# FireMines/zk_stark_project

Hardware: AMD Instinct MI355X
Metric: STARK proofs/sec + prove-time ms, MiMC AIR 2^20-step trace (higher is better)
Workload: dtype f128 (u128 mod 2^128-45*2^40+1); 1 GPU; MiMC AIR 2^20-step trace, blowup=8 (BASELINE configs[1]); trace_length=1048576, trace_width=1, blowup=8, num_queries=40, grinding=21, fri_folding=16, fri_remainder_max_degree=7, parallelism=replicas1

## Files before the change

zk_stark_project_amd/csrc/merkle.hip:

```cpp
#include "kernels_dev.hpp"
#include "blake3_quad.hpp"

#include <cstdlib>

using kc::rev_bits;
using kc::static_for;

namespace {

struct MerkleArgs {
  const felt* src;
  uint64_t n;
  uint32_t cols;
  uint32_t logB;
  uint64_t R;
  uint32_t* nodes;
  uint64_t L;
  MerkleTail tail;
  LastCol lc;
  GuLazy gl;
};

__device__ __forceinline__ felt gu_lazy_value(const GuLazy& gl, const felt* base, const felt* prev, uint64_t cstride,
                                              felt l, uint32_t c) {
// ... 183 lines not shown
      uint32_t l[8], r[8];
#pragma unroll
      for (int i = 0; i < 8; i++) { l[i] = sd[(2 * t) * 9 + i]; r[i] = sd[(2 * t + 1) * 9 + i]; }
      merge8(l, r, o);
    }
    __syncthreads();
    if (t < s) {
#pragma unroll
      for (int i = 0; i < 8; i++) sd[t * 9 + i] = o[i];
      store_digest(nodes + (first + t) * 8, o);
    }
  }
}

__device__ __forceinline__ void merkle_tail_op(const MerkleTail& tl, const uint32_t* root);

template <int MODE, bool QUAD = false>
__global__ __launch_bounds__(256) void k_merkle_fused(MerkleArgs a) {
  __shared__ uint32_t sd[256 * 9];
  const uint32_t t = threadIdx.x;
  const uint64_t L = a.L;
  constexpr uint64_t LB = QUAD ? 64 : 512;
  const uint64_t cnt = L < LB ? L : LB;
  const uint64_t base = (uint64_t)blockIdx.x * LB;
  uint64_t first;
  uint32_t s0;
  if constexpr (QUAD) {
    const uint32_t nd = t >> 2, q = t & 3;
    if (nd < cnt) {
      uint32_t o0, o1;
// ... 9 lines not shown
      merkle_leaf<MODE>(a, base + 2 * t, d0);
      merkle_leaf<MODE>(a, base + 2 * t + 1, d1);
      if (MODE != 2) {
        store_digest(a.nodes + (L + base + 2 * t) * 8, d0);
        store_digest(a.nodes + (L + base + 2 * t + 1) * 8, d1);
      }
      merge8(d0, d1, m);
      store_digest(a.nodes + ((L >> 1) + (base >> 1) + t) * 8, m);
#pragma unroll
      for (int i = 0; i < 8; i++) sd[t * 9 + i] = m[i];
    }
    first = (L >> 1) + (base >> 1);
    s0 = (uint32_t)(cnt >> 2);
  }
  lds_levels(sd, s0, a.nodes, first);
  if (!a.tail.done) return;
  __shared__ int s_last;
  __threadfence();
  __syncthreads();
  if (t == 0) s_last = atomicAdd(a.tail.done, 1u) == gridDim.x - 1;
  __syncthreads();
  if (!s_last) return;
  __threadfence();
  const uint32_t G = gridDim.x;
  if (G > 1) {
    if (G / 2 <= 64) {
      const uint32_t nd = t >> 2, q = t & 3;
      if (t < 4 * (G / 2)) {
        uint32_t mm[16], o0, o1;
        const uint32_t* src = a.nodes + (uint64_t)(G + 2 * nd) * 8;
#pragma unroll
        for (int k = 0; k < 16; k++) mm[k] = src[k];
        merge_quad(mm, q, o0, o1);
        quad_store(sd, a.nodes + (uint64_t)(G / 2 + nd) * 8, nd, q, o0, o1);
      }
    } else {
      for (uint32_t i = t; i < G / 2; i += 256) {
        uint32_t l[8], r[8], o[8];
        load_digest(a.nodes + (uint64_t)(G + 2 * i) * 8, l);
        load_digest(a.nodes + (uint64_t)(G + 2 * i + 1) * 8, r);
        merge8(l, r, o);
        store_digest(a.nodes + (uint64_t)(G / 2 + i) * 8, o);
#pragma unroll
        for (int k = 0; k < 8; k++) sd[i * 9 + k] = o[k];
      }
    }
    lds_levels(sd, G / 4, a.nodes, G / 2);
  }
  __syncthreads();
  if (t == 0) *a.tail.done = 0;
  if (a.tail.op != MERKLE_TAIL_NONE) merkle_tail_op(a.tail, a.nodes + 8);
}
// ... 382 lines not shown
  seed[4 + q] = s1;
  root_out[q] = r[q];
  root_out[4 + q] = r[4 + q];
}

__global__ void k_coin_fri_layer(uint32_t* __restrict__ seed, const uint32_t* __restrict__ root,
                                 felt* __restrict__ alpha_out, uint32_t* __restrict__ root_out) {
  if (blockIdx.x != 0) return;
  coin_fri_step(seed, root, alpha_out, root_out);
}

struct SeedArg {
  uint32_t w[8];
};

__global__ __launch_bounds__(TPB) void k_pack(PackArgs a, uint32_t* __restrict__ dst) {
  const uint32_t seg = blockIdx.y;
  if (seg >= a.n) return;
  const uint32_t* src = reinterpret_cast<const uint32_t*>(a.src[seg]);
  const uint64_t words = a.bytes[seg] / 4, o = a.off[seg] / 4;
  for (uint64_t i = blockIdx.x * (uint64_t)TPB + threadIdx.x; i < words; i += (uint64_t)gridDim.x * TPB)
    dst[o + i] = src[i];
}

__device__ __forceinline__ felt shfl_down_felt(felt v, int d) {
  const int a = __shfl_down((int)(uint32_t)v.lo, d), b = __shfl_down((int)(uint32_t)(v.lo >> 32), d);
  const int c = __shfl_down((int)(uint32_t)v.hi, d), e = __shfl_down((int)(uint32_t)(v.hi >> 32), d);
  return fp::make((uint64_t)(uint32_t)a | ((uint64_t)(uint32_t)b << 32),
                  (uint64_t)(uint32_t)c | ((uint64_t)(uint32_t)e << 32));
}
__device__ __forceinline__ void remainder_coeffs_block(const felt* __restrict__ E, uint32_t logB, uint32_t m,
                                                       uint32_t ncoef, felt off_inv, felt wd_inv, felt d_inv,
                                                       felt* s_c, felt* s_tw) {
  const uint32_t D = m << logB, t = threadIdx.x, lane = t & 63, wave = t >> 6, nw = blockDim.x >> 6;
  for (uint32_t j = t; j < D; j += blockDim.x) s_tw[j] = fp::pow_u64(wd_inv, j);
  __syncthreads();
  for (uint32_t k = wave; k < ncoef; k += nw) {
// ... 34 lines not shown
  uint32_t m[16];
#pragma unroll
  for (int k = 0; k < 8; k++) m[k] = seedp ? seedp[k] : seed.w[k];
  m[8] = (uint32_t)nonce;
  m[9] = (uint32_t)(nonce >> 32);
#pragma unroll
  for (int k = 10; k < 16; k++) m[k] = 0;
  uint32_t out[8];
  b3::set_iv(out);
  b3::compress(out, m, 0, 40, b3::CHUNK_START | b3::CHUNK_END | b3::ROOT);
  uint64_t h = (uint64_t)out[0] | ((uint64_t)out[1] << 32);
  uint32_t tz = h == 0 ? 64u : (uint32_t)__builtin_ctzll(h);
  if (tz >= bits) atomicMin(result, (unsigned long long)nonce);
}

__global__ __launch_bounds__(TPB) void k_grind_all(const uint32_t* __restrict__ seedp, uint64_t base, uint64_t limit,
                                                   uint32_t bits, unsigned long long* result) {
  const uint64_t T = (uint64_t)gridDim.x * TPB, g = blockIdx.x * (uint64_t)TPB + threadIdx.x;
  using b3::rotr;
  uint32_t m[16];
#pragma unroll
  for (int k = 0; k < 8; k++) m[k] = seedp[k];
#pragma unroll
  for (int k = 8; k < 16; k++) m[k] = 0;
  uint32_t p0 = b3::iv(0), p1 = b3::iv(1), p2 = b3::iv(2), p3 = b3::iv(3), p4 = b3::iv(4), p5 = b3::iv(5),
           p6 = b3::iv(6), p7 = b3::iv(7), p8 = b3::iv(0), p9 = b3::iv(1), p10 = b3::iv(2), p11 = b3::iv(3),
           p12 = 0, p13 = 0, p14 = 40, p15 = b3::CHUNK_START | b3::CHUNK_END | b3::ROOT;
  {
#define sp(i) p##i
#define B3_GP(a, b, c, d, x, y)            \
  sp(a) = sp(a) + sp(b) + (x);              \
  sp(d) = rotr(sp(d) ^ sp(a), 16);          \
  sp(c) = sp(c) + sp(d);                    \
  sp(b) = rotr(sp(b) ^ sp(c), 12);          \
  sp(a) = sp(a) + sp(b) + (y);              \
  sp(d) = rotr(sp(d) ^ sp(a), 8);           \
  sp(c) = sp(c) + sp(d);                    \
  sp(b) = rotr(sp(b) ^ sp(c), 7);
    B3_GP(0, 4, 8, 12, m[0], m[1]) B3_GP(1, 5, 9, 13, m[2], m[3])
    B3_GP(2, 6, 10, 14, m[4], m[5]) B3_GP(3, 7, 11, 15, m[6], m[7])
    B3_GP(1, 6, 11, 12, 0u, 0u) B3_GP(2, 7, 8, 13, 0u, 0u) B3_GP(3, 4, 9, 14, 0u, 0u)
#undef B3_GP
#undef sp
  }
  for (uint64_t start = base;; start += T) {
    if (start > limit || __hip_atomic_load(result, __ATOMIC_RELAXED, __HIP_MEMORY_SCOPE_AGENT) < start) return;
    const uint64_t nonce = start + g;
    m[8] = (uint32_t)nonce;
    m[9] = (uint32_t)(nonce >> 32);
    uint32_t s0 = p0, s1 = p1, s2 = p2, s3 = p3, s4 = p4, s5 = p5, s6 = p6, s7 = p7, s8 = p8, s9 = p9, s10 = p10,
             s11 = p11, s12 = p12, s13 = p13, s14 = p14, s15 = p15;
    B3_G(0, 5, 10, 15, m[8], m[9])
    B3_ROUND(2, 6, 3, 10, 7, 0, 4, 13, 1, 11, 12, 5, 9, 14, 15, 8)
    B3_ROUND(3, 4, 10, 12, 13, 2, 7, 14, 6, 5, 9, 0, 11, 15, 8, 1)
    B3_ROUND(10, 7, 12, 9, 14, 3, 13, 15, 4, 0, 11, 2, 5, 8, 1, 6)
    B3_ROUND(12, 13, 9, 11, 15, 10, 14, 8, 7, 2, 5, 3, 0, 1, 6, 4)
    B3_ROUND(9, 14, 11, 5, 8, 12, 15, 1, 13, 3, 0, 10, 2, 6, 4, 7)
    B3_ROUND(11, 15, 5, 0, 1, 9, 8, 6, 14, 10, 2, 12, 3, 4, 7, 13)
    const uint64_t h = (uint64_t)(s0 ^ s8) | ((uint64_t)(s1 ^ s9) << 32);
    const uint32_t tz = h == 0 ? 64u : (uint32_t)__builtin_ctzll(h);
    if (tz >= bits) atomicMin(result, (unsigned long long)nonce);
  }
}

__global__ void k_query_positions(const uint32_t* __restrict__ seedp, const unsigned long long* __restrict__ nonce_p,
                                  uint32_t q, uint64_t N, uint64_t* __restrict__ pos) {
  const uint64_t nonce = *nonce_p;
  uint32_t m[16], s2[8];
#pragma unroll
  for (int k = 0; k < 8; k++) m[k] = seedp[k];
  m[8] = (uint32_t)nonce;
  m[9] = (uint32_t)(nonce >> 32);
#pragma unroll
  for (int k = 10; k < 16; k++) m[k] = 0;
  b3::set_iv(s2);
  b3::compress_r(s2, m, 0, 40, b3::CHUNK_START | b3::CHUNK_END | b3::ROOT);
  for (uint32_t i = threadIdx.x; i < q; i += blockDim.x) {
#pragma unroll
    for (int k = 0; k < 8; k++) m[k] = s2[k];
    m[8] = i + 1;
    m[9] = 0;
#pragma unroll
    for (int k = 10; k < 16; k++) m[k] = 0;
    uint32_t out[8];
    b3::set_iv(out);
    b3::compress_r(out, m, 0, 40, b3::CHUNK_START | b3::CHUNK_END | b3::ROOT);
    pos[i] = ((uint64_t)out[0] | ((uint64_t)out[1] << 32)) & (N - 1);
  }
}

__global__ __launch_bounds__(128) void k_gather_full(FullGatherArgs a, const uint64_t* __restrict__ pos,
                                                     uint32_t* __restrict__ out) {
  const uint32_t i = blockIdx.x, y = blockIdx.y, t = threadIdx.x;
  const uint64_t p = pos[i];
  const uint64_t B = 1ull << a.logB;
  uint32_t* rec = out + a.seg_off[y] + (uint64_t)i * a.rec_words[y];
  if (y == 0) {
    const uint64_t j = p & (B - 1), tt = p >> a.logB;
    const uint32_t nv = a.w + a.C, depth = a.logN;
    for (uint32_t e = t; e < 4 * nv; e += blockDim.x) {
      const uint32_t c = e >> 2;
      const felt* src = c < a.w ? a.tlde + ((uint64_t)c * B + j) * a.n : a.clde + ((uint64_t)(c - a.w) * B + j) * a.n;
      rec[e] = reinterpret_cast<const uint32_t*>(src + tt)[e & 3];
    }
    uint32_t* paths = rec + 4 * nv;
    for (uint32_t e = t; e < 2 * depth * 8; e += blockDim.x) {
      const uint32_t tree = e / (depth * 8), d = (e / 8) % depth, wd = e & 7;
      const uint64_t node = (((1ull << a.logN) + p) >> d) ^ 1ull;
// ... 118 lines not shown
  const uint64_t q = tq >> 2;
  const uint32_t qd = (uint32_t)(tq & 3);
  const felt v = fri_fold_row_quad(E, q < rows ? q : rows - 1, qd, logm16, j0, logB, alpha_p, off_inv, itw_lev,
                                   eps_inv);
  if (q < rows && qd == 0) out[q] = v;
}

template <int F>
__global__ __launch_bounds__(TPB) void k_fri_fold(const felt* __restrict__ E, uint64_t rows, uint32_t logmF,
                                                  uint32_t j0, uint32_t logB, const felt* __restrict__ alpha_p,
                                                  felt off_inv, const felt* __restrict__ itw_lev,
                                                  const felt* __restrict__ eps_inv, felt* __restrict__ out) {
  const uint64_t q = blockIdx.x * (uint64_t)TPB + threadIdx.x;
  if (q >= rows) return;
  out[q] = fri_fold_row_f<F>(E, q, logmF, j0, logB, alpha_p, off_inv, itw_lev, eps_inv);
}

template <int F>
__global__ __launch_bounds__(512) void k_fri_tail(FriTailArgs a) {
  __shared__ uint32_t sd[128 * 9];
  __shared__ felt s_c[256];
  __shared__ felt s_tw[256];
  __shared__ uint32_t s_cv[32][8];
  const uint32_t t = threadIdx.x, nd = t >> 2, q = t & 3;
  for (uint32_t l = 0; l < a.nl; l++) {
    const FriTailLayer y = a.ly[l];
    const uint32_t R = 1u << (y.logm16 + a.logB);
    MerkleArgs ma{};
    ma.src = y.E;
    ma.R = 1ull << y.logm16;
// ... 142 lines not shown
void preload_merkle_module() {
  hipFuncAttributes fa;
  (void)hipFuncGetAttributes(&fa, (const void*)k_coin_fri_layer);
}

void launch_grind(Prof& prof, hipStream_t s, const uint32_t* seed_words, const uint32_t* seed_dev, uint64_t base,
                  uint64_t count, uint32_t bits, unsigned long long* result) {
  SeedArg sa;
  for (int i = 0; i < 8; i++) sa.w[i] = seed_words ? seed_words[i] : 0u;
  LAUNCH(prof, "grind", s, 0.0,
         hipLaunchKernelGGL(k_grind, dim3(blocks_for(count)), dim3(TPB), 0, s, sa, seed_dev, base, count, bits,
                            result));
}

void launch_grind_all(Prof& prof, hipStream_t s, const uint32_t* seed_dev, uint64_t base, uint64_t limit,
                      uint32_t bits, unsigned long long* result) {
  LAUNCH(prof, "grind", s, 0.0,
         hipLaunchKernelGGL(k_grind_all, dim3(1024), dim3(TPB), 0, s, seed_dev, base, limit, bits, result));
}

void launch_query_positions(Prof& prof, hipStream_t s, const uint32_t* seed_dev, const unsigned long long* nonce,
                            uint32_t q, uint64_t N, uint64_t* pos) {
  LAUNCH(prof, "positions", s, 0.0, hipLaunchKernelGGL(k_query_positions, dim3(1), dim3(256), 0, s, seed_dev, nonce, q,
                                                       N, pos));
}

void launch_gather_full(Prof& prof, hipStream_t s, const FullGatherArgs& a, uint32_t q, const uint64_t* pos,
                        uint32_t* out) {
  LAUNCH(prof, "gather", s, 0.0,
         hipLaunchKernelGGL(k_gather_full, dim3(q, 1 + a.nlayers), dim3(128), 0, s, a, pos, out));
}

void launch_pack(Prof& prof, hipStream_t s, const PackArgs& a, void* dst) {
  uint64_t mx = 0;
  for (uint32_t i = 0; i < a.n; i++) mx = a.bytes[i] > mx ? a.bytes[i] : mx;
  const uint32_t bx = (uint32_t)std::min<uint64_t>(std::max<uint64_t>((mx / 4 + TPB - 1) / TPB, 1), 64);
  LAUNCH(prof, "gather", s, 0.0,
         hipLaunchKernelGGL(k_pack, dim3(bx, a.n), dim3(TPB), 0, s, a, reinterpret_cast<uint32_t*>(dst)));
}

void launch_fri_remainder(Prof& prof, hipStream_t s, const felt* E, uint32_t logB, uint32_t m, felt off_inv,
                          felt wd_inv, felt d_inv, uint32_t* seed, felt* rem_out, uint32_t* commit_out) {
  const uint32_t D = m << logB, ncoef = m;
  if (D > 256) launch_fail(ZKP_ERR_DEVICE, "internal: device remainder over 256 values");
  LAUNCH(prof, "coin", s, 0.0,
// ... 15 lines not shown
  const uint64_t rows = m16 * Bl;
  if (F == 16 && rows <= (1ull << 15)) {
    LAUNCH(prof, "fri_fold16", s, (double)rows * (16 * 16.0 + 16.0),
           hipLaunchKernelGGL(k_fri_fold16_quad, dim3(blocks_for(rows * 4)), dim3(TPB), 0, s, E, rows, logm16, j0,
                              logB, alpha, off_inv, lev, eps_inv, out));
    return;
  }
#define ZKP_FOLD(FF)                                                                                             \
  case FF:                                                                                                       \
    LAUNCH(prof, "fri_fold" #FF, s, (double)rows * (FF * 16.0 + 16.0),                                           \
           hipLaunchKernelGGL(k_fri_fold<FF>, dim3(blocks_for(rows)), dim3(TPB), 0, s, E, rows, logm16, j0, logB, \
                              alpha, off_inv, lev, eps_inv, out));                                               \
    return;
  switch (F) { ZKP_FOLD(2) ZKP_FOLD(4) ZKP_FOLD(8) ZKP_FOLD(16) }
#undef ZKP_FOLD
  launch_fail(ZKP_ERR_DEVICE, "internal: FRI folding factor");
}

void launch_fri_tail(Prof& prof, hipStream_t s, const FriTailArgs& a) {
  if (a.nl > FRI_TAIL_MAX || (a.rem_m << a.logB) > 256) launch_fail(ZKP_ERR_DEVICE, "internal: FRI tail shape");
  for (uint32_t l = 0; l < a.nl; l++) {
    const uint32_t logrows = a.ly[l].logm16 + a.logB;
    if (logrows > 7)
      launch_fail(ZKP_ERR_DEVICE, "internal: FRI tail layer over 128 rows");
    if (logrows < 1) launch_fail(ZKP_ERR_DEVICE, "internal: FRI tail layer of one row");
  }
#define ZKP_TAIL(FF) \
  case FF: LAUNCH(prof, "fri_tail", s, 0.0, hipLaunchKernelGGL(k_fri_tail<FF>, dim3(1), dim3(512), 0, s, a)); return;
  switch (a.F) { ZKP_TAIL(2) ZKP_TAIL(4) ZKP_TAIL(8) ZKP_TAIL(16) }
#undef ZKP_TAIL
// ... 106 lines not shown
```

zk_stark_project_amd/csrc/prover.cpp:

```cpp
#include "prover_internal.hpp"

#include <mutex>

using namespace zkpi;

namespace zkpi {

int ProofRun::init(int air_id, const felt* d_trace_in, uint32_t width, uint64_t n_rows, const zkp_felt* pub_elems,
                   uint64_t n_pub, uint8_t** proof, uint64_t* proof_len) {
  d_trace = d_trace_in;
  w = width;
  n = n_rows;
  int rc = check_options(o);
  if (rc) return rc;
  if (n < 8 || (n & (n - 1)) || w == 0 || w > 255) return ZKP_ERR_TRACE_SHAPE;
  if (!proof || !proof_len || (n_pub && !pub_elems)) return ZKP_ERR_ARGUMENT;
  B = o->blowup_factor; F = o->fri_folding_factor;
  logn = ilog2(n); logB = ilog2(B); logN = logn + logB;
  N = 1ull << logN;
  if (logN > MAX_LOG_DOMAIN || logn > MAX_LOG_TRACE) return ZKP_ERR_TRACE_SHAPE;
  rc = check_fri_shape(n, o);
  if (rc) return rc;
  R = (uint32_t)cm->world; rank = (uint32_t)cm->rank;
  if (R == 0 || (R & (R - 1)) || R > B || rank >= R) return ZKP_ERR_ARGUMENT;
// ... 325 lines not shown
      felt* full = ctx->buf<felt>("fri_full_" + std::to_string(l), (size_t)B * m);
      cm->all_gather(st, E, full, (size_t)Bl * m * 16);
      E = full;
      Bc = B;
      jc = 0;
      sh = false;
    };
    uint32_t* coin_d = ctx->buf<uint32_t>("fri_coin", 8 + 12 * (size_t)(L + 1));
    felt* alphas_d = reinterpret_cast<felt*>(coin_d + 8);
    uint32_t* roots_d = coin_d + 8 + 4 * (size_t)L;
    HIP_CHECK(hipMemcpyAsync(coin_d, dt_seed, 32, hipMemcpyDeviceToDevice, st));
    static const bool no_fri_tail = getenv("ZKP_NO_FRI_TAIL") != nullptr;
    const bool fuse_tail = R == 1 && o->grinding_factor > 0 && (N >> (ilog2(F) * L)) <= 256 && !no_fri_tail;
    FriTailArgs fta{};
    fta.F = F;
    for (uint32_t l = 0; l < L; l++) {
      const uint64_t m16 = m / F;
      if (sh && (m16 >> logR) < 16) replicate(l);
      FriLayer& ly = layers[l];
      ly.E = E; ly.m = m; ly.Bc = Bc; ly.jc = jc; ly.sharded = sh;
      if (fuse_tail && (m16 << logB) <= 128) {
        if (fta.nl >= FRI_TAIL_MAX) throw ZkpFail{ZKP_ERR_DEVICE, "FRI tail: too many small layers"};
        ly.tree.logR = 0;
        ly.tree.Lr = m16 << logB;
        ly.tree.nodes = ctx->buf<uint32_t>("ftree_" + std::to_string(l), (size_t)16 * ly.tree.Lr);
        ly.tree.top.assign(2, {});
        FriTailLayer& y = fta.ly[fta.nl++];
        y.E = E;
        y.nodes = ly.tree.nodes;
        y.logm16 = ilog2(m16);
        y.off_inv = inv(off);
        y.lev = ctx->itws(logN) + ((1ull << (ilog2(D) - 1)) - 1);
        y.out = fe + eo;
        y.alpha_out = alphas_d + l;
        y.root_out = roots_d + 8 * (size_t)l;
        E = fe + eo;
        eo += (uint64_t)Bc * m16;
        m = m16;
        D /= F;
        off = pow_u64(off, F);
        continue;
      }
      if (fta.nl) throw ZkpFail{ZKP_ERR_DEVICE, "FRI tail: a large layer after a small one"};
      MerkleTail coin{};
      coin.op = MERKLE_TAIL_FRI_COIN;
      coin.coin_seed = coin_d;
      coin.alpha_out = alphas_d + l;
      coin.root_out = roots_d + 8 * (size_t)l;
      const bool coin_done = commit_rows(ctx, cm, 1, E, 0, F, logB, ilog2(m16), sh, "ftree_" + std::to_string(l),
                                         ly.tree, T.fri_roots[l], false, &coin);
      if (!coin_done)
        launch_coin_fri_layer(pf, st, coin_d, sh ? ly.tree.top_d + 8 : ly.tree.nodes + 8, alphas_d + l,
                              roots_d + 8 * (size_t)l);
      felt* nxt = fe + eo;
      launch_fri_fold(pf, st, E, m16, Bc, jc, logB, F, alphas_d + l, inv(off), ctx->itws(logN), ilog2(D), deps,
                      nxt);
      eo += (uint64_t)Bc * m16;
      E = nxt;
      m = m16;
      D /= F;
      off = pow_u64(off, F);
    }
    if (sh) replicate(L);
    layers[L].E = E; layers[L].m = m; layers[L].Bc = B; layers[L].jc = 0; layers[L].sharded = false;
    const uint64_t Dlast = (uint64_t)B * m;
    dev_tail = Dlast <= 256 && o->grinding_factor > 0;
    if (fuse_tail && !dev_tail) throw ZkpFail{ZKP_ERR_DEVICE, "FRI tail fused without a device remainder"};
    dev_query = dev_tail && R == 1 && L <= GATHER_MAX_LAYERS;
    if (dev_tail) {
      rem_d = ctx->buf<felt>("rem_d", m + 1);
      rcommit_d = ctx->buf<uint32_t>("rem_commit", 8);
// ... 2 lines not shown
        fta.coin_seed = coin_d;
        fta.eps_inv = deps;
        fta.rem_E = E;
        fta.rem_m = (uint32_t)m;
        fta.rem_off_inv = inv(off);
        fta.wd_inv = inv(root_of_unity(ilog2(Dlast)));
        fta.d_inv = inv(felt_u64(Dlast));
        fta.rem_out = rem_d;
        fta.commit_out = rcommit_d;
        launch_fri_tail(pf, st, fta);
      } else {
        launch_fri_remainder(pf, st, E, logB, (uint32_t)m, inv(off), inv(root_of_unity(ilog2(Dlast))),
                             inv(felt_u64(Dlast)), coin_d, rem_d, rcommit_d);
      }
      HIP_CHECK(hipMemsetAsync(dres, 0xff, 8, st));
      if (dev_query)
        launch_grind_all(pf, st, coin_d, 1, 1ull << 40, o->grinding_factor, dres);
      else
        launch_grind(pf, st, nullptr, coin_d, 1, grind_chunk, o->grinding_factor, dres);
    }
    if (dev_query) {
      dpos = ctx->buf<uint64_t>("query_pos", o->num_queries);
      launch_query_positions(pf, st, coin_d, dres, o->num_queries, N, dpos);
      ga.tlde = tlde; ga.clde = clde; ga.tnodes = ttree.nodes; ga.cnodes = ctree.nodes;
      ga.n = n; ga.w = w; ga.C = C; ga.logB = logB; ga.logN = logN; ga.nlayers = L; ga.F = F;
      uint64_t off_w = 0;
      ga.seg_off[0] = 0;
      ga.rec_words[0] = 4 * (w + C) + 16 * logN;
      off_w += (uint64_t)o->num_queries * ga.rec_words[0];
      for (uint32_t l = 0; l < L; l++) {
        ga.E[l] = layers[l].E;
        ga.fnodes[l] = layers[l].tree.nodes;
        ga.m[l] = layers[l].m;
        ga.logrows[l] = logB + ilog2(layers[l].m / F);
        ga.seg_off[1 + l] = off_w;
        ga.rec_words[1 + l] = 4 * F + 8 * ga.logrows[l];
        off_w += (uint64_t)o->num_queries * ga.rec_words[1 + l];
      }
      full_h.resize(off_w);
      uint32_t* dfull = ctx->buf<uint32_t>("query_full", off_w + 4);
      if (gu_lazy_on) launch_gu_fill(pf, st, tlde, w, logn, logB, j0, logBl, dpos, o->num_queries, gu_lazy);
      launch_gather_full(pf, st, ga, o->num_queries, dpos, dfull);
      raw_pos.resize(o->num_queries);
      full_d = dfull;
    }
    return FriCursor{E, m, D, off, coin_d, alphas_d, roots_d};
  }
}

void ProofRun::fri_round_trip(const FriCursor& c) {
  late_pairs_upload();
  felt* const E = c.E;
  const uint64_t m = c.m, D = c.D;
  const felt off = c.off;
  uint32_t* const coin_d = c.coin_d;
  felt* const alphas_d = c.alphas_d;
  uint32_t* const roots_d = c.roots_d;
  {
    std::vector<uint8_t> rb((size_t)L * 32);
    std::vector<felt> dalpha(L);
    std::vector<felt> cm_vals((size_t)B * m);
    std::vector<felt> dcc(ncoef), dzz(2), hood((size_t)2 * (w + C)), hgam(w + C), hdk(4);
    std::vector<felt> drem(dev_tail ? m : 0);
    uint8_t roots[64], drcommit[32], dseed[32];
    std::vector<Fetch> fs = {{dalpha.data(), alphas_d, (size_t)L * 16}, {rb.data(), roots_d, (size_t)L * 32},
                             {cm_vals.data(), E, cm_vals.size() * 16}, {dcc.data(), dt_cc, (size_t)ncoef * 16},
                             {dzz.data(), dt_zz, 32}, {hood.data(), dv, hood.size() * 16},
                             {hgam.data(), dgam, hgam.size() * 16}, {hdk.data(), dk, 64},
                             {roots, troot_d, 32}, {roots + 32, croot_d, 32}};
    if (dev_tail) {
      fs.push_back({drem.data(), rem_d, drem.size() * 16});
      fs.push_back({drcommit, rcommit_d, 32});
      fs.push_back({dseed, coin_d, 32});
      fs.push_back({&dnonce, dres, 8});
    }
    if (dev_query) {
      fs.push_back({raw_pos.data(), dpos, raw_pos.size() * 8});
      fs.push_back({full_h.data(), full_d, full_h.size() * 4});
    }
    for (TreeShard* t : {&ttree, &ctree})
      if (t->top_d) fs.push_back({t->top.data(), t->top_d, t->top.size() * 32});
    for (uint32_t l = 0; l < L; l++)
      if (layers[l].tree.top_d) fs.push_back({layers[l].tree.top.data(), layers[l].tree.top_d, layers[l].tree.top.size() * 32});
    fetch_all(ctx, fs);
    memcpy(T.trace_root, roots, 32);
    memcpy(T.constraint_root, roots + 32, 32);
    if (R == 1) {
      memcpy(ttree.top[1].data(), T.trace_root, 32);
      memcpy(ctree.top[1].data(), T.constraint_root, 32);
    }
    bool same = true;
    coin.reseed(T.trace_root);
    std::vector<felt> cc = draw_coeffs(coin, o->batching_constraints, ncoef);
    for (uint32_t i = 0; i < ncoef && same; i++) same = eq(cc[i], dcc[i]);
    coin.reseed(T.constraint_root);
    const felt z = coin.draw(), zg = mul(z, wn_root);
    same = same && eq(z, dzz[0]) && eq(zg, dzz[1]);
    T.z.lo = z.lo; T.z.hi = z.hi;
    for (uint32_t c = 0; c < w; c++) { ood_trace[c] = hood[2 * c]; ood_trace[w + c] = hood[2 * c + 1]; }
// ... 295 lines not shown
```

zk_stark_project_amd/csrc/prover_internal.hpp:

```cpp
#pragma once
#include <algorithm>
#include <array>
#include <chrono>
#include <cstdio>
#include <cstdlib>
#include <cstring>
#include <map>
#include <memory>
#include <stdexcept>
#include <string>
#include <utility>
#include <vector>

#include "../../include/zkp.h"
#include "blake3.hpp"
#include "comm.hpp"
#include "zkp_internal.hpp"

using namespace fp;

#include "host_stark.hpp"

using namespace zkh;

// ... 446 lines not shown
  const felt* twn = nullptr;
  const felt* d_trace = nullptr;
  felt *coef = nullptr, *tlde = nullptr, *comp = nullptr, *acoef = nullptr, *clde = nullptr;
  TreeShard ttree, ctree;
  const uint32_t *troot_d = nullptr, *croot_d = nullptr;
  felt wn_root{};
  felt *deep_inv = nullptr, *dv = nullptr, *dgam = nullptr, *dk = nullptr, *deep = nullptr;
  std::vector<felt> ood_trace, ood_comp;
  uint32_t L = 0;
  std::vector<FriLayer> layers;
  std::vector<felt> remainder;
  bool dev_tail = false;
  bool dev_query = false;
  FullGatherArgs ga{};
  uint64_t* dpos = nullptr;
  const uint32_t* full_d = nullptr;
  std::vector<uint32_t> full_h;
  std::vector<uint64_t> raw_pos;
  felt* rem_d = nullptr;
  uint32_t* rcommit_d = nullptr;
  unsigned long long* dres = nullptr;
  unsigned long long dnonce = ~0ull;
  static constexpr uint64_t grind_chunk = 1ull << 22;
  uint64_t nonce = 0;
  bool allow_shortcuts = true;
  bool paired = false;
  felt* gu_cval = nullptr;
  uint32_t* gu_bad = nullptr;
  uint32_t* gu_flags = nullptr;
  bool gu_lazy_on = false;
  bool gu_late_check = false;
// ... 40 lines not shown
  int finish(uint8_t** proof, uint64_t* proof_len, zkp_transcript* tr_out);
  void trace_column_sharded(const zkp_felt* h_trace, uint32_t cpt, uint32_t wi, uint32_t d);
  const zkp_felt* gather_host_slices(const zkp_felt* h_trace);
  felt* composition_exchange(felt* cint, uint64_t nR);
  void composition_gather_lde(felt* slice, bool derive, uint64_t nR, uint64_t p0);
};

bool commit_rows(zkp_ctx* ctx, zkp_comm* cm, int mode, const felt* src, uint64_t n, uint32_t cols, uint32_t logB,
                 uint32_t logrows, bool sharded, const std::string& name, TreeShard& tr, uint8_t root[32],
                 bool fetch_root = true, const MerkleTail* coin = nullptr, const LastCol* lc = nullptr,
                 const GuLazy* gl = nullptr);
bool commit_rows_sharded(zkp_ctx* ctx, zkp_comm* cm, int mode, const felt* src, uint64_t n, uint32_t cols,
                         uint32_t logB, uint32_t logrows, const std::string& name, TreeShard& tr, uint8_t root[32],
                         bool fetch_root, const MerkleTail* coin, const LastCol* lc, const GuLazy* gl);
void fetch_all(zkp_ctx* ctx, const std::vector<Fetch>& fs);
felt* ood_launch(zkp_ctx* ctx, const felt* arrays, uint32_t narrays, uint32_t ntwo, uint32_t logn, const felt* dpw,
                 zkp_comm* cm = nullptr);
felt* ood_launch_sharded(zkp_ctx* ctx, const felt* arrays, uint32_t narrays, uint32_t ntwo, uint32_t logn,
                         const felt* dpw, zkp_comm* cm, felt* part, felt* dv);
felt* coset_points(zkp_ctx* ctx, uint32_t logn, uint32_t logB, uint32_t logce);
const felt* coset_points8(zkp_ctx* ctx, uint32_t logn, uint32_t logB);
felt deep_ginv(uint32_t logn);
void constraint_eval(zkp_ctx* ctx, const AirDesc& air, uint32_t logn, uint32_t logB, uint32_t logce, uint32_t u0,
                     uint32_t cel, uint32_t j0, uint32_t logBl, const felt* cx, const felt* twn, const felt* dt_cc,
                     const felt* dt_aval, const felt* tlde, felt* comp, const felt* coef = nullptr,
                     zkp_comm* cm = nullptr);
const felt* last_col_kappa(zkp_ctx* ctx, uint32_t logn, uint32_t logB, uint32_t C);
std::vector<felt> comp_dft_consts(uint64_t n, uint32_t logce, uint32_t C);
void deep_evaluations(zkp_ctx* ctx, zkp_comm* cm, hipStream_t st, DeepArgs da, const felt* coef, uint64_t n,
                      const felt* Sj0, uint32_t logN, felt* out);
// ... 44 lines not shown
```

zk_stark_project_amd/csrc/prover_stages.cpp:

```cpp
#include "prover_internal.hpp"

using namespace zkpi;

namespace zkpi {

bool commit_rows(zkp_ctx* ctx, zkp_comm* cm, int mode, const felt* src, uint64_t n, uint32_t cols, uint32_t logB,
                 uint32_t logrows, bool sharded, const std::string& name, TreeShard& tr, uint8_t root[32],
                 bool fetch_root, const MerkleTail* coin, const LastCol* lc, const GuLazy* gl) {
  Prof& pf = ctx->prof;
  hipStream_t st = ctx->stream;
  const uint64_t L = 1ull << (logB + logrows);
  if (!sharded) {
    tr.logR = 0;
    tr.Lr = L;
    tr.nodes = ctx->buf<uint32_t>(name, (size_t)16 * L);
    uint32_t* done = ctx->buf<uint32_t>("merkle_done", 1);
    if (!ctx->have_cached("merkle_done")) HIP_CHECK(hipMemsetAsync(done, 0, 4, st));
    MerkleTail tail = coin ? *coin : MerkleTail{};
    tail.done = done;
    bool ran = mode == 0 ? launch_merkle_lde(pf, st, src, cols, logB, n, tr.nodes, L, &tail, lc, gl)
                         : launch_merkle_fri(pf, st, src, 1ull << logrows, logB, cols, tr.nodes, &tail);
    tr.top.assign(2, {});
    if (fetch_root) {
      ctx->download(root, tr.nodes + 8, 32);
      memcpy(tr.top[1].data(), root, 32);
    }
    return ran && coin;
  }
  return commit_rows_sharded(ctx, cm, mode, src, n, cols, logB, logrows, name, tr, root, fetch_root, coin, lc, gl);
}

void fetch_all(zkp_ctx* ctx, const std::vector<Fetch>& fs) {
  size_t tot = 0;
  for (const Fetch& f : fs) tot += (f.bytes + 15) & ~(size_t)15;
  uint8_t* hp = (uint8_t*)ctx->pinned(tot + 16);
  uint8_t* stage = ctx->buf<uint8_t>("fetch_stage", tot + 16);
  size_t o = 0;
  PackArgs pa{};
  auto flush = [&] {
    if (pa.n) launch_pack(ctx->prof, ctx->stream, pa, stage);
    pa.n = 0;
  };
  for (const Fetch& f : fs) {
    if (f.bytes % 4) throw ZkpFail{ZKP_ERR_ARGUMENT, "fetch of a non-word-sized segment"};
    if (f.bytes) {
      pa.src[pa.n] = f.dev;
      pa.bytes[pa.n] = f.bytes;
      pa.off[pa.n] = o;
      if (++pa.n == PACK_MAX) flush();
    }
    o += (f.bytes + 15) & ~(size_t)15;
  }
  flush();
  HIP_CHECK(hipMemcpyAsync(hp, stage, tot, hipMemcpyDeviceToHost, ctx->stream));
  ctx->sync();
  o = 0;
  for (const Fetch& f : fs) {
    memcpy(f.host, hp + o, f.bytes);
    o += (f.bytes + 15) & ~(size_t)15;
  }
}

felt* ood_launch(zkp_ctx* ctx, const felt* arrays, uint32_t narrays, uint32_t ntwo, uint32_t logn,
                 const felt* dpw, zkp_comm* cm) {
  uint32_t logE = logn < 11 ? logn : 11;
  if (logn - logE > 12) throw ZkpFail{ZKP_ERR_TRACE_SHAPE, "OOD evaluation supports n <= 2^23"};
  const uint32_t nb = 1u << (logn - logE);
  felt* part = ctx->buf<felt>("ood_part", (size_t)2 * narrays * nb);
  felt* dv = ctx->buf<felt>("ood_vals", (size_t)2 * narrays);
  const felt ninv = inv(felt_u64(1ull << logn));
  const uint32_t R = cm ? (uint32_t)cm->world : 1u;
  if (R == 1 || nb < R) {
    launch_eval_bitrev(ctx->prof, ctx->stream, arrays, narrays, ntwo, logn, dpw, dpw + logn, part, ninv, dv);
    return dv;
  }
  return ood_launch_sharded(ctx, arrays, narrays, ntwo, logn, dpw, cm, part, dv);
// ... 556 lines not shown
```

zk_stark_project_amd/csrc/zkp_internal.hpp:

```cpp
#pragma once
#include <hip/hip_runtime.h>
#include <stdint.h>

#include <string>
#include <vector>

#include "felt.hpp"
#include "pcg64.hpp"

struct ProfRec {
  const char* name;
  double bytes;
  hipEvent_t start, stop;
};
struct Prof {
  bool enabled = false;
  std::string only;
  bool open = false;
  std::vector<ProfRec> pending;
  std::vector<hipEvent_t> pool;
  hipEvent_t get_event();
  void begin(const char* name, hipStream_t s, double bytes);
  void end(hipStream_t s);
};
// ... 57 lines not shown
                      const MerkleTail* tail);
void launch_merkle_from_shards(Prof& prof, hipStream_t s, const uint32_t* recv, uint32_t logB, uint32_t logrr,
                               uint32_t logK, uint32_t* nodes, uint32_t* done = nullptr);
constexpr uint32_t PACK_MAX = 16;
struct PackArgs {
  const void* src[PACK_MAX];
  uint64_t bytes[PACK_MAX], off[PACK_MAX];
  uint32_t n;
};
void launch_pack(Prof& prof, hipStream_t s, const PackArgs& a, void* dst);
void launch_grind(Prof& prof, hipStream_t s, const uint32_t* seed_words, const uint32_t* seed_dev, uint64_t base,
                  uint64_t count, uint32_t bits, unsigned long long* result);
void launch_fri_remainder(Prof& prof, hipStream_t s, const felt* E, uint32_t logB, uint32_t m, felt off_inv,
                          felt wd_inv, felt d_inv, uint32_t* seed, felt* rem_out, uint32_t* commit_out);

void launch_grind_all(Prof& prof, hipStream_t s, const uint32_t* seed_dev, uint64_t base, uint64_t limit,
                      uint32_t bits, unsigned long long* result);
void launch_query_positions(Prof& prof, hipStream_t s, const uint32_t* seed_dev, const unsigned long long* nonce,
                            uint32_t q, uint64_t N, uint64_t* pos);
constexpr uint32_t GATHER_MAX_LAYERS = 16;
struct FullGatherArgs {
  const felt* tlde;
  const felt* clde;
  const uint32_t* tnodes;
  const uint32_t* cnodes;
  uint64_t n;
  uint32_t w, C, logB, logN, nlayers;
  uint32_t F;
  const felt* E[GATHER_MAX_LAYERS];
  const uint32_t* fnodes[GATHER_MAX_LAYERS];
  uint64_t m[GATHER_MAX_LAYERS];
  uint32_t logrows[GATHER_MAX_LAYERS];
  uint64_t seg_off[GATHER_MAX_LAYERS + 1];
  uint32_t rec_words[GATHER_MAX_LAYERS + 1];
};
void launch_gather_full(Prof& prof, hipStream_t s, const FullGatherArgs& a, uint32_t q, const uint64_t* pos,
                        uint32_t* out);

void launch_dt_draw_coeffs(Prof& prof, hipStream_t s, uint32_t* seed, const uint32_t* root, uint32_t method,
                           uint32_t ncoef, felt* cc);
void launch_dt_eval_consts(Prof& prof, hipStream_t s, int air, const felt* cc, felt k, felt w_last, const felt* aval,
                           const felt* zinv, uint32_t ce, uint32_t w, uint32_t num_t, felt* out);
void launch_dt_deep_coeffs(Prof& prof, hipStream_t s, uint32_t* seed, const felt* ood, uint32_t w, uint32_t C,
                           uint32_t method, felt* gamma, felt* dk);
void launch_dt_draw_z(Prof& prof, hipStream_t s, uint32_t* seed, const uint32_t* root, felt wn, uint32_t logn,
                      felt* zz, felt* pw);

void launch_gu_trace(Prof& prof, hipStream_t s, const felt* masked, const felt* raw, const felt* local,
                     uint64_t ndev, felt kinv, uint64_t n, felt* tile_buf, felt* out);
struct TuClient {
  felt* out;
  const uint64_t* masks;
// ... 165 lines not shown
struct DeepRoots {
  felt w8, w8_2, w8_3;
};
inline uint64_t deep_den_scratch(uint64_t count) { return count / 8 + count / (8 * 2048) + 2; }
void launch_deep_denominators(Prof& prof, hipStream_t s, hipStream_t s2, hipEvent_t ev, const PointMap& m,
                              const PointMap& m8, const DeepRoots& r, uint64_t count, const felt* zz, const felt* pw,
                              felt* scratch, felt* table);
void launch_deep(Prof& prof, hipStream_t s, const DeepArgs& a, felt* out);
void launch_deep_lincomb(Prof& prof, hipStream_t s, const felt* coef, uint32_t w, uint64_t n, uint64_t p0,
                         uint64_t np, const felt* gamma, felt* out,
                         felt* scratch);

void launch_fri_fold(Prof& prof, hipStream_t s, const felt* E, uint64_t m16, uint32_t Bl, uint32_t j0,
                     uint32_t logB, uint32_t F, const felt* alpha, felt off_inv, const felt* itw, uint32_t logD,
                     const felt* eps_inv_dev, felt* out);
constexpr uint32_t FRI_TAIL_MAX = 7;
struct FriTailLayer {
  const felt* E;
  uint32_t* nodes;
  uint32_t logm16;
  felt off_inv;
  const felt* lev;
  felt* out;
  felt* alpha_out;
  uint32_t* root_out;
};
struct FriTailArgs {
  uint32_t nl, logB, F;
  FriTailLayer ly[FRI_TAIL_MAX];
  uint32_t* coin_seed;
// ... 23 lines not shown
```

Measured before the change: 233.1 proofs/s.

## Fuse FRI fold with next-layer Merkle commit, grind with query positions, gather with pack

Adds a kernel that folds an FRI layer and builds the next layer's Merkle tree plus the coin draw in one launch, using a last-block-done counter. It also moves query-position derivation into the last block of the grind kernel, and merges the final gather with the fetch pack into one launch. Host pair upload now overlaps the async fetch. The aim is fewer kernel launches and fewer global round trips on the serial FRI/query tail. In exchange the code carries more atomic-counter state, and the fused fold kernel runs at 1024 threads with a fixed grid limit.

```diff
diff --git a/zk_stark_project_amd/csrc/merkle.hip b/zk_stark_project_amd/csrc/merkle.hip
--- a/zk_stark_project_amd/csrc/merkle.hip
+++ b/zk_stark_project_amd/csrc/merkle.hip
@@ -221,6 +221,7 @@
 }
 
 __device__ __forceinline__ void merkle_tail_op(const MerkleTail& tl, const uint32_t* root);
+__device__ __forceinline__ void merkle_finish_block(const MerkleArgs& a, uint32_t* sd);
 
 template <int MODE, bool QUAD = false>
 __global__ __launch_bounds__(256) void k_merkle_fused(MerkleArgs a) {
@@ -260,6 +261,11 @@
     s0 = (uint32_t)(cnt >> 2);
   }
   lds_levels(sd, s0, a.nodes, first);
+  merkle_finish_block(a, sd);
+}
+
+__device__ __forceinline__ void merkle_finish_block(const MerkleArgs& a, uint32_t* sd) {
+  const uint32_t t = threadIdx.x;
   if (!a.tail.done) return;
   __shared__ int s_last;
   __threadfence();
@@ -281,7 +287,7 @@
         quad_store(sd, a.nodes + (uint64_t)(G / 2 + nd) * 8, nd, q, o0, o1);
       }
     } else {
-      for (uint32_t i = t; i < G / 2; i += 256) {
+      for (uint32_t i = t; i < G / 2; i += blockDim.x) {
         uint32_t l[8], r[8], o[8];
         load_digest(a.nodes + (uint64_t)(G + 2 * i) * 8, l);
         load_digest(a.nodes + (uint64_t)(G + 2 * i + 1) * 8, r);
@@ -694,13 +700,15 @@
   uint32_t w[8];
 };
 
-__global__ __launch_bounds__(TPB) void k_pack(PackArgs a, uint32_t* __restrict__ dst) {
-  const uint32_t seg = blockIdx.y;
+__device__ __forceinline__ void pack_segment(const PackArgs& a, uint32_t seg, uint32_t* __restrict__ dst) {
   if (seg >= a.n) return;
   const uint32_t* src = reinterpret_cast<const uint32_t*>(a.src[seg]);
   const uint64_t words = a.bytes[seg] / 4, o = a.off[seg] / 4;
-  for (uint64_t i = blockIdx.x * (uint64_t)TPB + threadIdx.x; i < words; i += (uint64_t)gridDim.x * TPB)
+  for (uint64_t i = blockIdx.x * (uint64_t)blockDim.x + threadIdx.x; i < words; i += (uint64_t)gridDim.x * blockDim.x)
     dst[o + i] = src[i];
+}
+__global__ __launch_bounds__(TPB) void k_pack(PackArgs a, uint32_t* __restrict__ dst) {
+  pack_segment(a, blockIdx.y, dst);
 }
 
 __device__ __forceinline__ felt shfl_down_felt(felt v, int d) {
@@ -765,8 +773,11 @@
   if (tz >= bits) atomicMin(result, (unsigned long long)nonce);
 }
 
+__device__ __forceinline__ void query_positions_block(const uint32_t* __restrict__ seedp, uint64_t nonce, uint32_t q,
+                                                      uint64_t N, uint64_t* __restrict__ pos);
+
 __global__ __launch_bounds__(TPB) void k_grind_all(const uint32_t* __restrict__ seedp, uint64_t base, uint64_t limit,
-                                                   uint32_t bits, unsigned long long* result) {
+                                                   uint32_t bits, unsigned long long* result, GrindTail tl) {
   const uint64_t T = (uint64_t)gridDim.x * TPB, g = blockIdx.x * (uint64_t)TPB + threadIdx.x;
   using b3::rotr;
   uint32_t m[16];
@@ -795,7 +806,7 @@
 #undef sp
   }
   for (uint64_t start = base;; start += T) {
-    if (start > limit || __hip_atomic_load(result, __ATOMIC_RELAXED, __HIP_MEMORY_SCOPE_AGENT) < start) return;
+    if (start > limit || __hip_atomic_load(result, __ATOMIC_RELAXED, __HIP_MEMORY_SCOPE_AGENT) < start) break;
     const uint64_t nonce = start + g;
     m[8] = (uint32_t)nonce;
     m[9] = (uint32_t)(nonce >> 32);
@@ -812,11 +823,21 @@
     const uint32_t tz = h == 0 ? 64u : (uint32_t)__builtin_ctzll(h);
     if (tz >= bits) atomicMin(result, (unsigned long long)nonce);
   }
-}
-
-__global__ void k_query_positions(const uint32_t* __restrict__ seedp, const unsigned long long* __restrict__ nonce_p,
-                                  uint32_t q, uint64_t N, uint64_t* __restrict__ pos) {
-  const uint64_t nonce = *nonce_p;
+  if (!tl.done) return;
+  __shared__ int s_last;
+  __threadfence();
+  __syncthreads();
+  if (threadIdx.x == 0) s_last = atomicAdd(tl.done, 1u) == gridDim.x - 1;
+  __syncthreads();
+  if (!s_last) return;
+  __threadfence();
+  if (threadIdx.x == 0) *tl.done = 0;
+  query_positions_block(seedp, __hip_atomic_load(result, __ATOMIC_RELAXED, __HIP_MEMORY_SCOPE_AGENT), tl.q, tl.N,
+                        tl.pos);
+}
+
+__device__ __forceinline__ void query_positions_block(const uint32_t* __restrict__ seedp, uint64_t nonce, uint32_t q,
+                                                      uint64_t N, uint64_t* __restrict__ pos) {
   uint32_t m[16], s2[8];
 #pragma unroll
   for (int k = 0; k < 8; k++) m[k] = seedp[k];
@@ -841,8 +862,13 @@
 }
 
 __global__ __launch_bounds__(128) void k_gather_full(FullGatherArgs a, const uint64_t* __restrict__ pos,
-                                                     uint32_t* __restrict__ out) {
+                                                     uint32_t* __restrict__ out, PackArgs pk,
+                                                     uint32_t* __restrict__ stage) {
   const uint32_t i = blockIdx.x, y = blockIdx.y, t = threadIdx.x;
+  if (y > a.nlayers) {
+    pack_segment(pk, y - a.nlayers - 1, stage);
+    return;
+  }
   const uint64_t p = pos[i];
   const uint64_t B = 1ull << a.logB;
   uint32_t* rec = out + a.seg_off[y] + (uint64_t)i * a.rec_words[y];
@@ -991,6 +1017,45 @@
   const uint64_t q = blockIdx.x * (uint64_t)TPB + threadIdx.x;
   if (q >= rows) return;
   out[q] = fri_fold_row_f<F>(E, q, logmF, j0, logB, alpha_p, off_inv, itw_lev, eps_inv);
+}
+
+template <int F>
+__global__ __launch_bounds__(1024) void k_fri_fold_commit(const felt* __restrict__ E, uint32_t logmF,
+                                                          const felt* __restrict__ alpha_p, felt off_inv,
+                                                          const felt* __restrict__ itw_lev,
+                                                          const felt* __restrict__ eps_inv, felt* __restrict__ out,
+                                                          MerkleArgs a) {
+  constexpr uint32_t LB = 1024 / F, SDN = LB > 256 ? LB : 256;
+  __shared__ felt s_val[1024];
+  __shared__ uint32_t sd[SDN * 9];
+  const uint32_t t = threadIdx.x;
+  const uint64_t L = a.L;
+  const uint32_t cnt = L < LB ? (uint32_t)L : LB;
+  const uint64_t base = (uint64_t)blockIdx.x * LB;
+  {
+    const uint32_t kk = t / LB, r = t % LB;
+    const uint32_t B = 1u << a.logB;
+    const uint32_t T = cnt >> a.logB;
+    const uint32_t li = T ? ((r % T) << a.logB) | (r / T) : r;
+    if (r < cnt && (T == 0 || r / T < B)) {
+      const uint64_t i = base + li;
+      const uint64_t q = ((i & (B - 1)) << logmF) + (uint64_t)kk * a.R + (i >> a.logB);
+      const felt v = fri_fold_row_f<F>(E, q, logmF, 0, a.logB, alpha_p, off_inv, itw_lev, eps_inv);
+      out[q] = v;
+      s_val[kk * LB + li] = v;
+    }
+  }
+  __syncthreads();
+  MerkleArgs la{};
+  la.src = s_val;
+  la.R = LB;
+  for (uint32_t nd = t >> 2; nd < cnt; nd += blockDim.x >> 2) {
+    uint32_t o0, o1;
+    fri_leaf_quad<F>(la, nd, t & 3, o0, o1);
+    quad_store(sd, a.nodes + (L + base + nd) * 8, nd, t & 3, o0, o1);
+  }
+  lds_levels(sd, cnt >> 1, a.nodes, L + base);
+  merkle_finish_block(a, sd);
 }
 
 template <int F>
@@ -1163,21 +1228,21 @@
 }
 
 void launch_grind_all(Prof& prof, hipStream_t s, const uint32_t* seed_dev, uint64_t base, uint64_t limit,
-                      uint32_t bits, unsigned long long* result) {
+                      uint32_t bits, unsigned long long* result, const GrindTail* tail) {
+  const GrindTail tl = tail ? *tail : GrindTail{};
   LAUNCH(prof, "grind", s, 0.0,
-         hipLaunchKernelGGL(k_grind_all, dim3(1024), dim3(TPB), 0, s, seed_dev, base, limit, bits, result));
-}
-
-void launch_query_positions(Prof& prof, hipStream_t s, const uint32_t* seed_dev, const unsigned long long* nonce,
-                            uint32_t q, uint64_t N, uint64_t* pos) {
-  LAUNCH(prof, "positions", s, 0.0, hipLaunchKernelGGL(k_query_positions, dim3(1), dim3(256), 0, s, seed_dev, nonce, q,
-                                                       N, pos));
+         hipLaunchKernelGGL(k_grind_all, dim3(1024), dim3(TPB), 0, s, seed_dev, base, limit, bits, result,
+                            tl));
 }
 
 void launch_gather_full(Prof& prof, hipStream_t s, const FullGatherArgs& a, uint32_t q, const uint64_t* pos,
-                        uint32_t* out) {
+                        uint32_t* out, const PackArgs* pack, void* stage) {
+  const PackArgs pk = pack ? *pack : PackArgs{};
+  if (q == 0 || a.nlayers > GATHER_MAX_LAYERS || pk.n > PACK_MAX || (pk.n && !stage))
+    launch_fail(ZKP_ERR_DEVICE, "internal: gather launch shape");
   LAUNCH(prof, "gather", s, 0.0,
-         hipLaunchKernelGGL(k_gather_full, dim3(q, 1 + a.nlayers), dim3(128), 0, s, a, pos, out));
+         hipLaunchKernelGGL(k_gather_full, dim3(q, 1 + a.nlayers + pk.n), dim3(128), 0, s, a, pos, out, pk,
+                            reinterpret_cast<uint32_t*>(stage)));
 }
 
 void launch_pack(Prof& prof, hipStream_t s, const PackArgs& a, void* dst) {
@@ -1223,6 +1288,40 @@
     return;
   switch (F) { ZKP_FOLD(2) ZKP_FOLD(4) ZKP_FOLD(8) ZKP_FOLD(16) }
 #undef ZKP_FOLD
+  launch_fail(ZKP_ERR_DEVICE, "internal: FRI folding factor");
+}
+
+bool fri_fold_commit_fits(uint64_t m16, uint32_t logB, uint32_t F) {
+  if (m16 < F || m16 % F) return false;
+  const uint64_t L = (m16 / F) << logB, LB = 1024 / F;
+  return L >= 2 && (L + LB - 1) / LB <= 512;
+}
+
+void launch_fri_fold_commit(Prof& prof, hipStream_t s, const felt* E, uint64_t m16, uint32_t logB, uint32_t F,
+                            const felt* alpha, felt off_inv, const felt* itw, uint32_t logD, const felt* eps_inv,
+                            felt* out, uint32_t* nodes, const MerkleTail& tail) {
+  if (!fri_fold_commit_fits(m16, logB, F) || !tail.done)
+    launch_fail(ZKP_ERR_DEVICE, "internal: fused fold and commitment shape");
+  const felt* lev = itw + ((1ull << (logD - 1)) - 1);
+  const uint32_t logm16 = kc::ilog2_u64(m16);
+  MerkleArgs a{};
+  a.R = m16 / F;
+  a.logB = logB;
+  a.cols = F;
+  a.nodes = nodes;
+  a.L = a.R << logB;
+  a.tail = tail;
+  const uint64_t LB = 1024 / F;
+  const dim3 g((uint32_t)((a.L + LB - 1) / LB));
+  const double bytes = (double)(m16 << logB) * (F * 16.0 + 16.0) + (double)a.L * 64.0;
+#define ZKP_FOLDC(FF)                                                                                            \
+  case FF:                                                                                                       \
+    LAUNCH(prof, "fri_fold" #FF, s, bytes,                                                                  \
+           hipLaunchKernelGGL(k_fri_fold_commit<FF>, g, dim3(1024), 0, s, E, logm16, alpha, off_inv, lev, eps_inv, \
+                              out, a));                                                                          \
+    return;
+  switch (F) { ZKP_FOLDC(2) ZKP_FOLDC(4) ZKP_FOLDC(8) ZKP_FOLDC(16) }
+#undef ZKP_FOLDC
   launch_fail(ZKP_ERR_DEVICE, "internal: FRI folding factor");
 }
 
diff --git a/zk_stark_project_amd/csrc/prover.cpp b/zk_stark_project_amd/csrc/prover.cpp
--- a/zk_stark_project_amd/csrc/prover.cpp
+++ b/zk_stark_project_amd/csrc/prover.cpp
@@ -363,6 +363,10 @@
     const bool fuse_tail = R == 1 && o->grinding_factor > 0 && (N >> (ilog2(F) * L)) <= 256 && !no_fri_tail;
     FriTailArgs fta{};
     fta.F = F;
+    static const bool no_fold_commit = getenv("ZKP_NO_FOLD_COMMIT") != nullptr;
+    static const uint64_t fold_commit_max_rows =
+        getenv("ZKP_FOLD_COMMIT_MAX_LOG") ? 1ull << atoi(getenv("ZKP_FOLD_COMMIT_MAX_LOG")) : ~0ull;
+    bool committed = false;
     for (uint32_t l = 0; l < L; l++) {
       const uint64_t m16 = m / F;
       if (sh && (m16 >> logR) < 16) replicate(l);
@@ -391,19 +395,41 @@
         continue;
       }
       if (fta.nl) throw ZkpFail{ZKP_ERR_DEVICE, "FRI tail: a large layer after a small one"};
-      MerkleTail coin{};
-      coin.op = MERKLE_TAIL_FRI_COIN;
-      coin.coin_seed = coin_d;
-      coin.alpha_out = alphas_d + l;
-      coin.root_out = roots_d + 8 * (size_t)l;
-      const bool coin_done = commit_rows(ctx, cm, 1, E, 0, F, logB, ilog2(m16), sh, "ftree_" + std::to_string(l),
-                                         ly.tree, T.fri_roots[l], false, &coin);
-      if (!coin_done)
-        launch_coin_fri_layer(pf, st, coin_d, sh ? ly.tree.top_d + 8 : ly.tree.nodes + 8, alphas_d + l,
-                              roots_d + 8 * (size_t)l);
+      auto coin_of = [&](uint32_t layer) {
+        MerkleTail coin{};
+        coin.op = MERKLE_TAIL_FRI_COIN;
+        coin.coin_seed = coin_d;
+        coin.alpha_out = alphas_d + layer;
+        coin.root_out = roots_d + 8 * (size_t)layer;
+        return coin;
+      };
+      if (!committed) {
+        const MerkleTail coin = coin_of(l);
+        const bool coin_done = commit_rows(ctx, cm, 1, E, 0, F, logB, ilog2(m16), sh, "ftree_" + std::to_string(l),
+                                           ly.tree, T.fri_roots[l], false, &coin);
+        if (!coin_done)
+          launch_coin_fri_layer(pf, st, coin_d, sh ? ly.tree.top_d + 8 : ly.tree.nodes + 8, alphas_d + l,
+                                roots_d + 8 * (size_t)l);
+      }
       felt* nxt = fe + eo;
-      launch_fri_fold(pf, st, E, m16, Bc, jc, logB, F, alphas_d + l, inv(off), ctx->itws(logN), ilog2(D), deps,
-                      nxt);
+      const uint64_t next_rows = (m16 / F) << logB;
+      committed = !no_fold_commit && !sh && R == 1 && l + 1 < L && !(fuse_tail && next_rows <= 128) &&
+                  next_rows <= fold_commit_max_rows && fri_fold_commit_fits(m16, logB, F);
+      if (committed) {
+        TreeShard& nt = layers[l + 1].tree;
+        nt.logR = 0;
+        nt.Lr = next_rows;
+        nt.nodes = ctx->buf<uint32_t>("ftree_" + std::to_string(l + 1), (size_t)16 * next_rows);
+        nt.top.assign(2, {});
+        MerkleTail coin = coin_of(l + 1);
+        coin.done = ctx->buf<uint32_t>("merkle_done", 1);
+        if (!ctx->have_cached("merkle_done")) HIP_CHECK(hipMemsetAsync(coin.done, 0, 4, st));
+        launch_fri_fold_commit(pf, st, E, m16, logB, F, alphas_d + l, inv(off), ctx->itws(logN), ilog2(D), deps, nxt,
+                               nt.nodes, coin);
+      } else {
+        launch_fri_fold(pf, st, E, m16, Bc, jc, logB, F, alphas_d + l, inv(off), ctx->itws(logN), ilog2(D), deps,
+                        nxt);
+      }
       eo += (uint64_t)Bc * m16;
       E = nxt;
       m = m16;
@@ -436,14 +462,17 @@
                              inv(felt_u64(Dlast)), coin_d, rem_d, rcommit_d);
       }
       HIP_CHECK(hipMemsetAsync(dres, 0xff, 8, st));
-      if (dev_query)
-        launch_grind_all(pf, st, coin_d, 1, 1ull << 40, o->grinding_factor, dres);
-      else
+      if (dev_query) {
+        dpos = ctx->buf<uint64_t>("query_pos", o->num_queries);
+        uint32_t* done = ctx->buf<uint32_t>("grind_done", 1);
+        if (!ctx->have_cached("grind_done")) HIP_CHECK(hipMemsetAsync(done, 0, 4, st));
+        const GrindTail gt{done, dpos, N, o->num_queries};
+        launch_grind_all(pf, st, coin_d, 1, 1ull << 40, o->grinding_factor, dres, &gt);
+      } else {
         launch_grind(pf, st, nullptr, coin_d, 1, grind_chunk, o->grinding_factor, dres);
+      }
     }
     if (dev_query) {
-      dpos = ctx->buf<uint64_t>("query_pos", o->num_queries);
-      launch_query_positions(pf, st, coin_d, dres, o->num_queries, N, dpos);
       ga.tlde = tlde; ga.clde = clde; ga.tnodes = ttree.nodes; ga.cnodes = ctree.nodes;
       ga.n = n; ga.w = w; ga.C = C; ga.logB = logB; ga.logN = logN; ga.nlayers = L; ga.F = F;
       uint64_t off_w = 0;
@@ -460,18 +489,14 @@
         off_w += (uint64_t)o->num_queries * ga.rec_words[1 + l];
       }
       full_h.resize(off_w);
-      uint32_t* dfull = ctx->buf<uint32_t>("query_full", off_w + 4);
       if (gu_lazy_on) launch_gu_fill(pf, st, tlde, w, logn, logB, j0, logBl, dpos, o->num_queries, gu_lazy);
-      launch_gather_full(pf, st, ga, o->num_queries, dpos, dfull);
       raw_pos.resize(o->num_queries);
-      full_d = dfull;
     }
     return FriCursor{E, m, D, off, coin_d, alphas_d, roots_d};
   }
 }
 
 void ProofRun::fri_round_trip(const FriCursor& c) {
-  late_pairs_upload();
   felt* const E = c.E;
   const uint64_t m = c.m, D = c.D;
   const felt off = c.off;
@@ -496,15 +521,16 @@
       fs.push_back({dseed, coin_d, 32});
       fs.push_back({&dnonce, dres, 8});
     }
-    if (dev_query) {
-      fs.push_back({raw_pos.data(), dpos, raw_pos.size() * 8});
-      fs.push_back({full_h.data(), full_d, full_h.size() * 4});
-    }
+    if (dev_query) fs.push_back({raw_pos.data(), dpos, raw_pos.size() * 8});
     for (TreeShard* t : {&ttree, &ctree})
       if (t->top_d) fs.push_back({t->top.data(), t->top_d, t->top.size() * 32});
     for (uint32_t l = 0; l < L; l++)
       if (layers[l].tree.top_d) fs.push_back({layers[l].tree.top.data(), layers[l].tree.top_d, layers[l].tree.top.size() * 32});
-    fetch_all(ctx, fs);
+    const FetchGather fg{&ga, o->num_queries, dpos, full_h.data(), full_h.size()};
+    const FetchPlan plan = fetch_launch(ctx, fs, dev_query ? &fg : nullptr);
+    late_pairs_upload();
+    fetch_wait(ctx, plan);
+    ctx->stage_end("5a_fri_fetch");
     memcpy(T.trace_root, roots, 32);
     memcpy(T.constraint_root, roots + 32, 32);
     if (R == 1) {
diff --git a/zk_stark_project_amd/csrc/prover_internal.hpp b/zk_stark_project_amd/csrc/prover_internal.hpp
--- a/zk_stark_project_amd/csrc/prover_internal.hpp
+++ b/zk_stark_project_amd/csrc/prover_internal.hpp
@@ -484,7 +484,6 @@
   bool dev_query = false;
   FullGatherArgs ga{};
   uint64_t* dpos = nullptr;
-  const uint32_t* full_d = nullptr;
   std::vector<uint32_t> full_h;
   std::vector<uint64_t> raw_pos;
   felt* rem_d = nullptr;
@@ -555,6 +554,20 @@
                          uint32_t logB, uint32_t logrows, const std::string& name, TreeShard& tr, uint8_t root[32],
                          bool fetch_root, const MerkleTail* coin, const LastCol* lc, const GuLazy* gl);
 void fetch_all(zkp_ctx* ctx, const std::vector<Fetch>& fs);
+struct FetchGather {
+  const FullGatherArgs* ga;
+  uint32_t q;
+  const uint64_t* pos;
+  uint32_t* host;
+  size_t words;
+};
+struct FetchPlan {
+  std::vector<Fetch> fs;
+  uint8_t* hp = nullptr;
+  size_t tot = 0;
+};
+FetchPlan fetch_launch(zkp_ctx* ctx, const std::vector<Fetch>& fs, const FetchGather* g = nullptr);
+void fetch_wait(zkp_ctx* ctx, const FetchPlan& pl);
 felt* ood_launch(zkp_ctx* ctx, const felt* arrays, uint32_t narrays, uint32_t ntwo, uint32_t logn, const felt* dpw,
                  zkp_comm* cm = nullptr);
 felt* ood_launch_sharded(zkp_ctx* ctx, const felt* arrays, uint32_t narrays, uint32_t ntwo, uint32_t logn,
diff --git a/zk_stark_project_amd/csrc/prover_stages.cpp b/zk_stark_project_amd/csrc/prover_stages.cpp
--- a/zk_stark_project_amd/csrc/prover_stages.cpp
+++ b/zk_stark_project_amd/csrc/prover_stages.cpp
@@ -30,11 +30,14 @@
   return commit_rows_sharded(ctx, cm, mode, src, n, cols, logB, logrows, name, tr, root, fetch_root, coin, lc, gl);
 }
 
-void fetch_all(zkp_ctx* ctx, const std::vector<Fetch>& fs) {
-  size_t tot = 0;
-  for (const Fetch& f : fs) tot += (f.bytes + 15) & ~(size_t)15;
-  uint8_t* hp = (uint8_t*)ctx->pinned(tot + 16);
-  uint8_t* stage = ctx->buf<uint8_t>("fetch_stage", tot + 16);
+FetchPlan fetch_launch(zkp_ctx* ctx, const std::vector<Fetch>& fs, const FetchGather* g) {
+  FetchPlan pl;
+  pl.fs = fs;
+  size_t seg_bytes = 0;
+  for (const Fetch& f : fs) seg_bytes += (f.bytes + 15) & ~(size_t)15;
+  pl.tot = seg_bytes + (g ? g->words * 4 : 0);
+  pl.hp = (uint8_t*)ctx->pinned(pl.tot + 16);
+  uint8_t* stage = ctx->buf<uint8_t>("fetch_stage", pl.tot + 16);
   size_t o = 0;
   PackArgs pa{};
   auto flush = [&] {
@@ -44,22 +47,35 @@
   for (const Fetch& f : fs) {
     if (f.bytes % 4) throw ZkpFail{ZKP_ERR_ARGUMENT, "fetch of a non-word-sized segment"};
     if (f.bytes) {
+      if (pa.n == PACK_MAX) flush();
       pa.src[pa.n] = f.dev;
       pa.bytes[pa.n] = f.bytes;
       pa.off[pa.n] = o;
-      if (++pa.n == PACK_MAX) flush();
+      pa.n++;
     }
     o += (f.bytes + 15) & ~(size_t)15;
   }
-  flush();
-  HIP_CHECK(hipMemcpyAsync(hp, stage, tot, hipMemcpyDeviceToHost, ctx->stream));
+  if (g) {
+    launch_gather_full(ctx->prof, ctx->stream, *g->ga, g->q, g->pos, reinterpret_cast<uint32_t*>(stage + seg_bytes),
+                       &pa, stage);
+    pl.fs.push_back({g->host, nullptr, g->words * 4});
+  } else {
+    flush();
+  }
+  HIP_CHECK(hipMemcpyAsync(pl.hp, stage, pl.tot, hipMemcpyDeviceToHost, ctx->stream));
+  return pl;
+}
+
+void fetch_wait(zkp_ctx* ctx, const FetchPlan& pl) {
   ctx->sync();
-  o = 0;
-  for (const Fetch& f : fs) {
-    memcpy(f.host, hp + o, f.bytes);
+  size_t o = 0;
+  for (const Fetch& f : pl.fs) {
+    memcpy(f.host, pl.hp + o, f.bytes);
     o += (f.bytes + 15) & ~(size_t)15;
   }
 }
+
+void fetch_all(zkp_ctx* ctx, const std::vector<Fetch>& fs) { fetch_wait(ctx, fetch_launch(ctx, fs)); }
 
 felt* ood_launch(zkp_ctx* ctx, const felt* arrays, uint32_t narrays, uint32_t ntwo, uint32_t logn,
                  const felt* dpw, zkp_comm* cm) {
diff --git a/zk_stark_project_amd/csrc/zkp_internal.hpp b/zk_stark_project_amd/csrc/zkp_internal.hpp
--- a/zk_stark_project_amd/csrc/zkp_internal.hpp
+++ b/zk_stark_project_amd/csrc/zkp_internal.hpp
@@ -95,10 +95,14 @@
 void launch_fri_remainder(Prof& prof, hipStream_t s, const felt* E, uint32_t logB, uint32_t m, felt off_inv,
                           felt wd_inv, felt d_inv, uint32_t* seed, felt* rem_out, uint32_t* commit_out);
 
+struct GrindTail {
+  uint32_t* done;
+  uint64_t* pos;
+  uint64_t N;
+  uint32_t q;
+};
 void launch_grind_all(Prof& prof, hipStream_t s, const uint32_t* seed_dev, uint64_t base, uint64_t limit,
-                      uint32_t bits, unsigned long long* result);
-void launch_query_positions(Prof& prof, hipStream_t s, const uint32_t* seed_dev, const unsigned long long* nonce,
-                            uint32_t q, uint64_t N, uint64_t* pos);
+                      uint32_t bits, unsigned long long* result, const GrindTail* tail = nullptr);
 constexpr uint32_t GATHER_MAX_LAYERS = 16;
 struct FullGatherArgs {
   const felt* tlde;
@@ -116,7 +120,7 @@
   uint32_t rec_words[GATHER_MAX_LAYERS + 1];
 };
 void launch_gather_full(Prof& prof, hipStream_t s, const FullGatherArgs& a, uint32_t q, const uint64_t* pos,
-                        uint32_t* out);
+                        uint32_t* out, const PackArgs* pack = nullptr, void* stage = nullptr);
 
 void launch_dt_draw_coeffs(Prof& prof, hipStream_t s, uint32_t* seed, const uint32_t* root, uint32_t method,
                            uint32_t ncoef, felt* cc);
@@ -312,6 +316,10 @@
 void launch_fri_fold(Prof& prof, hipStream_t s, const felt* E, uint64_t m16, uint32_t Bl, uint32_t j0,
                      uint32_t logB, uint32_t F, const felt* alpha, felt off_inv, const felt* itw, uint32_t logD,
                      const felt* eps_inv_dev, felt* out);
+bool fri_fold_commit_fits(uint64_t m16, uint32_t logB, uint32_t F);
+void launch_fri_fold_commit(Prof& prof, hipStream_t s, const felt* E, uint64_t m16, uint32_t logB, uint32_t F,
+                            const felt* alpha, felt off_inv, const felt* itw, uint32_t logD, const felt* eps_inv_dev,
+                            felt* out, uint32_t* nodes, const MerkleTail& tail);
 constexpr uint32_t FRI_TAIL_MAX = 7;
 struct FriTailLayer {
   const felt* E;
```

Result: slower. 223.1 proofs/s (-4.3%).
